# joeyee/Onet

Measured on AMD Instinct MI355X. Metric: training images/sec (twin 256x256 pass), higher is better.
Workload: dtype f32

## Files before the change

### onet_amd/csrc/conv_split.hip

```cpp
#include <algorithm>
#include <cstdlib>
#include "common.hpp"

using namespace onet;

typedef float f32x16 __attribute__((ext_vector_type(16)));
typedef __bf16 bf16x8 __attribute__((ext_vector_type(8)));
typedef __bf16 bf16x2 __attribute__((ext_vector_type(2)));
typedef unsigned int u32x4s __attribute__((ext_vector_type(4)));
typedef float f32x4s __attribute__((ext_vector_type(4)));

namespace {

constexpr unsigned OOB_S = 0x80000000u;

__device__ __forceinline__ __amdgpu_buffer_rsrc_t s_rsrc(const void* base, int64_t bytes) {
    const int n = bytes > 0x7fffffffll ? 0x7fffffff : (int)bytes;
    return __builtin_amdgcn_make_buffer_rsrc(const_cast<void*>(base), 0, n, 0x00020000);
}
__device__ __forceinline__ void split2(float a, float b, unsigned& hi, unsigned& mid) {
    const bf16x2 h = {(__bf16)a, (__bf16)b};
    const bf16x2 m = {(__bf16)(a - (float)h[0]), (__bf16)(b - (float)h[1])};
    hi = __builtin_bit_cast(unsigned, h);
    mid = __builtin_bit_cast(unsigned, m);
// ... 358 lines not shown
                (void)tap;
#pragma unroll
                for (int m = 0; m < 2; ++m)
#pragma unroll
                    for (int n = 0; n < NT; ++n) {
                        if constexpr (F16) {
                            const f16x8 ah = __builtin_bit_cast(f16x8, Aq[idx & 1][m][0]), am = __builtin_bit_cast(f16x8, Aq[idx & 1][m][1]);
                            const f16x8 bh = __builtin_bit_cast(f16x8, Bq[kx & 1][n + ky][0]), bm = __builtin_bit_cast(f16x8, Bq[kx & 1][n + ky][1]);
                            acc[m][n] = __builtin_amdgcn_mfma_f32_32x32x16_f16(am, bh, acc[m][n], 0, 0, 0);
                            acc[m][n] = __builtin_amdgcn_mfma_f32_32x32x16_f16(ah, bm, acc[m][n], 0, 0, 0);
                            acc[m][n] = __builtin_amdgcn_mfma_f32_32x32x16_f16(ah, bh, acc[m][n], 0, 0, 0);
                        } else {
                            const bf16x8 ah = __builtin_bit_cast(bf16x8, Aq[idx & 1][m][0]), am = __builtin_bit_cast(bf16x8, Aq[idx & 1][m][1]);
                            const bf16x8 bh = __builtin_bit_cast(bf16x8, Bq[kx & 1][n + ky][0]), bm = __builtin_bit_cast(bf16x8, Bq[kx & 1][n + ky][1]);
                            acc[m][n] = __builtin_amdgcn_mfma_f32_32x32x16_bf16(am, bh, acc[m][n], 0, 0, 0);
                            acc[m][n] = __builtin_amdgcn_mfma_f32_32x32x16_bf16(ah, bm, acc[m][n], 0, 0, 0);
                            acc[m][n] = __builtin_amdgcn_mfma_f32_32x32x16_bf16(ah, bh, acc[m][n], 0, 0, 0);
                        }
                    }
                __builtin_amdgcn_sched_barrier(0);
            }
            __syncthreads();
            buf ^= 1;
        }

        if constexpr (F16) {
#pragma unroll
            for (int m = 0; m < 2; ++m)
#pragma unroll
                for (int n = 0; n < NT; ++n)
#pragma unroll
                    for (int r = 0; r < 16; ++r) acc[m][n][r] *= acc_scale;
        }
        const auto [co0, tx, ty, b, y0, x0] = sp_tile(tile, a.coTiles, a.tilesX, a.tilesY);
        if constexpr (ST) {
            float* sc = reinterpret_cast<float*>(lds + 2 * BUF);
            constexpr float npw = (float)(NT * 32), inv_npw = 1.f / npw;
#pragma unroll
            for (int m = 0; m < 2; ++m)
#pragma unroll
                for (int r = 0; r < 16; ++r) {
                    const int piv = __builtin_bit_cast(int, acc[m][0][r]);
                    const float p0 = __builtin_bit_cast(float, __builtin_amdgcn_readlane(piv, 0));
                    const float p1 = __builtin_bit_cast(float, __builtin_amdgcn_readlane(piv, 32));
                    const float pv = kh ? p1 : p0;
                    float s1 = 0.f, s2 = 0.f;
#pragma unroll
                    for (int n = 0; n < NT; ++n) {
                        const float d = acc[m][n][r] - pv;
                        s1 += d;
                        s2 = fmaf(d, d, s2);
                    }
                    s1 = sp_half_sum(s1);
                    s2 = sp_half_sum(s2);
                    if (l31 == 31) {
                        const int cl = m * 32 + (r & 3) + 8 * (r >> 2) + 4 * kh;
                        sc[(wn * 64 + cl) * 2] = fmaf(s1, inv_npw, pv);
                        sc[(wn * 64 + cl) * 2 + 1] = fmaxf(fmaf(-s1 * inv_npw, s1, s2), 0.f);
                    }
                }
            __syncthreads();
            if (tid < 64 && co0 + tid < a.Cout) {
                float mw[8], qw[8];
#pragma unroll
                for (int w = 0; w < 8; ++w) {
                    mw[w] = sc[(w * 64 + tid) * 2];
                    qw[w] = sc[(w * 64 + tid) * 2 + 1];
                }
                const float mean = 0.125f * (((mw[0] + mw[1]) + (mw[2] + mw[3])) + ((mw[4] + mw[5]) + (mw[6] + mw[7])));
                float m2 = ((qw[0] + qw[1]) + (qw[2] + qw[3])) + ((qw[4] + qw[5]) + (qw[6] + qw[7]));
#pragma unroll
                for (int w = 0; w < 8; ++w) m2 = fmaf(npw * (mw[w] - mean), mw[w] - mean, m2);
                const int64_t nblk = (int64_t)a.B * a.tilesY * a.tilesX;
                const int64_t blk = ((int64_t)b * a.tilesY + ty) * a.tilesX + tx;
                float* sp = a.stats + ((int64_t)(co0 + tid) * nblk + blk) * 3;
                sp[0] = 8.f * npw;
                sp[1] = mean;
                sp[2] = m2;
            }
            __syncthreads();
        }
        float* zb = a.z + (int64_t)b * a.z_bs;
        const int xo = x0 + l31;
#pragma unroll
        for (int m = 0; m < 2; ++m)
#pragma unroll
            for (int n = 0; n < NT; ++n) {
                const int yo = y0 + wn * NT + n;
                if (yo < a.H && xo < a.W) {
#pragma unroll
                    for (int r = 0; r < 16; ++r) {
                        const int co = co0 + m * 32 + (r & 3) + 8 * (r >> 2) + 4 * kh;
                        if (co < a.Cout) zb[(int64_t)co * HW + (int64_t)yo * a.W + xo] = acc[m][n][r];
                    }
                }
            }
    }
}


typedef int i32x4s __attribute__((ext_vector_type(4)));
__device__ __forceinline__ i32x4s sp_rsrc4(const void* base, int64_t bytes) {
    const uint64_t p = reinterpret_cast<uint64_t>(base);
    i32x4s r;
    r.x = (int)(p & 0xffffffffu);
    r.y = (int)((p >> 32) & 0xffffu);
    r.z = bytes > 0x7fffffffll ? 0x7fffffff : (int)bytes;
    r.w = 0x00020000;
    return r;
}
__device__ __forceinline__ void sp_dma16(i32x4s rsrc, unsigned lds_base, unsigned voff, unsigned soff) {
    unsigned keep;
    asm volatile("s_nop 4\n\ts_mov_b32 %0, m0\n\ts_mov_b32 m0, %3\n\ts_nop 0\n\tbuffer_load_dwordx4 %1, %2, %4 offen lds\n\ts_mov_b32 m0, %0"
                 : "=&s"(keep)
                 : "v"(voff), "s"(rsrc), "s"(lds_base), "s"(soff)
                 : "memory");
}

__global__ void split_pack_act_kernel(const float* __restrict__ x, int64_t x_bs, unsigned* __restrict__ xs, int64_t xs_bs, int B, int C8,
                                      int H, int W, int f16, float scale, const unsigned* __restrict__ slots) {
    if (slots) {
        float inv;
        scale *= amax_scale(amax_read(slots), false, inv);
    }
    const int64_t n = (int64_t)B * C8 * H * W;
    for (int64_t i = blockIdx.x * (int64_t)blockDim.x + threadIdx.x; i < n; i += (int64_t)gridDim.x * blockDim.x) {
        const int xx = (int)(i % W);
        int64_t r = i / W;
        const int y = (int)(r % H);
        r /= H;
        const int c8 = (int)(r % C8), b = (int)(r / C8);
        const float* src = x + (int64_t)b * x_bs + ((int64_t)c8 * 8 * H + y) * W + xx;
        u32x4s hi, mid;
#pragma unroll
        for (int c = 0; c < 4; ++c) {
            const float va = src[(int64_t)(2 * c) * H * W] * scale, vb = src[(int64_t)(2 * c + 1) * H * W] * scale;
            unsigned h, m;
            if (f16 == 1) split2h(va, vb, h, m);
            else split2(va, vb, h, m);
            hi[c] = h;
            mid[c] = m;
        }
        if (f16 == 2) {
            reinterpret_cast<u32x4s*>(xs + (int64_t)b * xs_bs)[((int64_t)c8 * H + y) * W + xx] = hi;
            continue;
        }
        u32x4s* dst = reinterpret_cast<u32x4s*>(xs + (int64_t)b * xs_bs) + (((int64_t)c8 * H + y) * 2) * W + xx;
        dst[0] = hi;
        dst[W] = mid;
    }
}

struct SpPreArgs {
    const void* xs;
    int64_t xs_bs;
    const __bf16* wq;
    float* z;
    int64_t z_bs;
    int B, Cin, Cout, H, W, tilesX, tilesY, coTiles;
    float* stats;
    const unsigned* x_slots;
    int x_always;
    const unsigned* x_slots2;
    int split_ch;
    const float* rd_z = nullptr;
    int64_t rd_z_bs = 0;
    const float* rd_save = nullptr;
    int rd_gimg = 0;
    float* rd_rec = nullptr;
    unsigned* rd_amax = nullptr;
    int z16 = 0, rd_z16 = 0;
    void* zP = nullptr;
    int64_t zP_bs = 0;
    int zP_ch0 = 0;
    const unsigned* zP_slots = nullptr;
    const float* act_save = nullptr;
    unsigned* act_amax = nullptr;
    float* act_a = nullptr;
    int64_t act_a_bs = 0;
    const float* hd_L = nullptr;
    int64_t hd_L_bs = 0;
    float* hd_V = nullptr;
};

template <bool W16> struct SpPreCfg {
    static constexpr int NW = 8, NT = 16 / NW, TW = 32, CO_T = 64, ROWS = NW * NT;
    static constexpr int IN_ROWS = ROWS + 2, IN_COLS = W16 ? 36 : 34;
    static constexpr int NPIX = IN_ROWS * IN_COLS;
    static constexpr int NPIXP = W16 ? 656 : 640;
    static constexpr int W_PART = 9 * 2 * CO_T, W_SLOTS = 2 * W_PART, NWI = (W_SLOTS + NW * 64 - 1) / (NW * 64);
    static constexpr int IN_PART = 2 * NPIXP;
    static constexpr int BUF_SLOTS = W_SLOTS + 2 * IN_PART;
    static constexpr int LDS_BYTES = 2 * BUF_SLOTS * 16;
    static constexpr int NB = (NT - 1) + 3;
    static constexpr int LAST_TAP = 4;
    static_assert(CO_T == SpCfg::CO_T && ROWS == SpCfg::ROWS && TW == SpCfg::TW, "sp_tile: one tile shape for every kernel of the family");
};
template <bool ST, int PM, bool W16, bool ACT = false>
__global__ __launch_bounds__(SpPreCfg<W16>::NW * 64, SpPreCfg<W16>::NW / 4) void conv3x3_split_pre_kernel(SpPreArgs a) {
    constexpr bool F16 = PM == 1;
    static_assert(!ACT || (PM == 1 && !ST && !W16), "conv3x3_split_pre_kernel: the activation epilogue goes with the fp16 slot store");
    using C = SpPreCfg<W16>;
    constexpr int NT = C::NT, IN_COLS = C::IN_COLS, NWI = C::NWI, CO_T = C::CO_T, NPIXP = C::NPIXP, NB = C::NB;
    constexpr int BUF = C::BUF_SLOTS, W_PART = C::W_PART, IN_PART = C::IN_PART;
    constexpr int NWV = C::NW, NTH = NWV * 64;
    constexpr int NII = (2 * IN_PART + NTH - 1) / NTH;
    extern __shared__ __attribute__((aligned(16))) unsigned char smem_s[];
    u32x4s* lds = reinterpret_cast<u32x4s*>(smem_s);

    int t_first, t_end, t_stride;
    sp_tile_range(a.tilesX * a.tilesY * a.B * a.coTiles, t_first, t_end, t_stride);
    if (t_first >= t_end) return;

    const int tid = threadIdx.x, lane = tid & 63, wn = __builtin_amdgcn_readfirstlane(tid >> 6);
    const int l31 = lane & 31, kh = lane >> 5;
    const int HW = a.H * a.W;
    const int nchunks = PM == 2 ? a.Cin >> 5 : a.Cin >> 4;

    const i32x4s wr = sp_rsrc4(a.wq, (int64_t)a.Cin * (PM == 2 ? 1 : 2) * 9 * a.Cout * 2);
    float xs_inv = 1.f, xs_inv2 = 1.f;
    (void)amax_scale(amax_read(a.x_slots), a.x_always != 0, xs_inv);
    (void)amax_scale(amax_read(a.x_slots2), a.x_always != 0, xs_inv2);
    const int split_chunk = a.split_ch ? (PM == 2 ? a.split_ch >> 5 : a.split_ch >> 4) : 0;
    const float grp_ratio = split_chunk ? xs_inv / xs_inv2 : 1.f;
    const float acc_scale = (split_chunk ? xs_inv2 : xs_inv) * (F16 ? reinterpret_cast<const float*>(a.wq + (int64_t)a.Cin * 2 * 9 * a.Cout)[1] : 1.f);
    const unsigned in_step = (unsigned)(16 * HW * 4), w_step = (unsigned)(2 * 9 * 2 * a.Cout * 16);
    const unsigned lds0 = (unsigned)(uintptr_t)(__attribute__((address_space(3))) unsigned char*)smem_s;

    unsigned in_off[NII], w_off[NWI];
    i32x4s xr;
    int st_tile = t_first, st_chunk = 0;
    unsigned cin_bytes = 0, cw_bytes = 0;
    auto setup_stage = [&]() __attribute__((always_inline)) {
        const bool live = st_tile < t_end;
        const auto [co0, tx, ty, b, y0, x0] = sp_tile(live ? st_tile : t_first, a.coTiles, a.tilesX, a.tilesY);
        xr = sp_rsrc4(reinterpret_cast<const unsigned*>(a.xs) + (int64_t)(W16 ? 2 * b : b) * a.xs_bs,
                      (W16 ? a.xs_bs * 4 : 0) + (int64_t)a.Cin * HW * (PM == 2 ? 2 : 4));
#pragma unroll
        for (int k = 0; k < NII; ++k) {
            const int i = (wn + NWV * k) * 64 + lane;
            const int ph = i / NPIXP, pix = i % NPIXP;
            const int r = pix / IN_COLS, c = pix % IN_COLS;
            const int img = W16 ? c / 18 : 0;
            const int yy = y0 - 1 + r, xx = W16 ? c % 18 - 1 : x0 - 1 + c;
            const bool ok = live && i < 2 * IN_PART && pix < C::NPIX && yy >= 0 && yy < a.H && xx >= 0 && xx < a.W;
            const unsigned io = W16 ? (unsigned)(img * a.xs_bs * 4) : 0u;
            in_off[k] = !ok ? OOB_S : PM == 2 ? io + (unsigned)(((ph * a.H + yy) * a.W + xx) * 16)
                                              : io + (unsigned)(((((ph & 1) * a.H + yy) * 2 + (ph >> 1)) * a.W + xx) * 16);
        }
#pragma unroll
        for (int k = 0; k < NWI; ++k) {
            const int i = tid + NTH * k;
            const int co = i & (CO_T - 1), pth = i >> 6;
            const bool ok = live && (i < C::W_SLOTS) && (co0 + co < a.Cout);
            w_off[k] = ok ? (unsigned)((pth * a.Cout + co0 + co) * 16) : OOB_S;
        }
    };
    auto advance = [&]() __attribute__((always_inline)) {
        ++st_chunk;
        cin_bytes += in_step;
        cw_bytes += w_step;
        if (st_chunk == nchunks) {
            st_chunk = 0;
            cin_bytes = cw_bytes = 0;
            st_tile += t_stride;
            setup_stage();
        }
    };
    auto dma_in = [&](int buf, int k) __attribute__((always_inline)) {
        if ((wn + NWV * k) * 64 < 2 * IN_PART)
            sp_dma16(xr, lds0 + (unsigned)((buf * BUF + C::W_SLOTS + (wn + NWV * k) * 64) * 16), in_off[k], cin_bytes);
    };
    auto dma_w = [&](int buf, int k) __attribute__((always_inline)) {
        if (k < NWI - 1 || wn < (C::W_SLOTS - NTH * (NWI - 1)) / 64)
            sp_dma16(wr, lds0 + (unsigned)((buf * BUF + (wn + NWV * k) * 64) * 16), w_off[k], cw_bytes);
    };

    const u32x4s* const a_ptr = lds + kh * CO_T + l31;
    const u32x4s* const b_ptr = lds + C::W_SLOTS + kh * NPIXP + (wn * NT) * IN_COLS + (W16 ? (l31 >> 4) * 18 + (l31 & 15) : l31);

    setup_stage();
#pragma unroll
    for (int k = 0; k < NII; ++k) dma_in(0, k);
#pragma unroll
    for (int k = 0; k < NWI; ++k) dma_w(0, k);
    asm volatile("s_waitcnt vmcnt(0)" ::: "memory");
    __syncthreads();
    int buf = 0;
    float zP_scale = 1.f;
    if constexpr (PM == 1 && !ST && !W16) {
        float zinv;
        if (a.zP) zP_scale = amax_scale(amax_read(a.zP_slots), !ACT, zinv);
    }
    [[maybe_unused]] float* const act_cf = reinterpret_cast<float*>(lds + 2 * BUF);
    [[maybe_unused]] float cf_next = 0.f;
    [[maybe_unused]] int cf_par = 0;
    auto act_fetch = [&](int t) __attribute__((always_inline)) {
        if (tid < 192 && t < t_end) {
            const int k = tid >> 6;
            cf_next = a.act_save[(int64_t)(k + (k > 0)) * a.Cout + sp_tile(t, a.coTiles, a.tilesX, a.tilesY).co0 + (tid & 63)];
        }
    };
    if constexpr (ACT) act_fetch(t_first);
    for (int tile = t_first; tile < t_end; tile += t_stride) {
        if constexpr (ACT) {
            cf_par ^= 1;
            if (tid < 192) act_cf[cf_par * 192 + tid] = cf_next;
            act_fetch(tile + t_stride);
        }
        f32x16 acc[2][NT];
#pragma unroll
        for (int m = 0; m < 2; ++m)
#pragma unroll
            for (int n = 0; n < NT; ++n)
#pragma unroll
                for (int r = 0; r < 16; ++r) acc[m][n][r] = 0.f;

        for (int c = 0; c < nchunks; ++c) {
            if (split_chunk && c == split_chunk && grp_ratio != 1.f) {
#pragma unroll
                for (int m = 0; m < 2; ++m)
#pragma unroll
                    for (int n = 0; n < NT; ++n)
#pragma unroll
                        for (int r = 0; r < 16; ++r) acc[m][n][r] *= grp_ratio;
            }
            const u32x4s* const ab = a_ptr + buf * BUF;
            const u32x4s* const bb = b_ptr + buf * BUF;
            u32x4s Aq[2][2][2], Bq[2][NB][2];
#pragma unroll
            for (int j = 0; j < NB; ++j) {
                Bq[0][j][0] = bb[j * IN_COLS];
                Bq[0][j][1] = bb[j * IN_COLS + IN_PART];
            }
#pragma unroll
            for (int m = 0; m < 2; ++m) {
                Aq[0][m][0] = ab[m * 32];
                Aq[0][m][1] = ab[m * 32 + W_PART];
            }
#pragma unroll
            for (int idx = 0; idx < 9; ++idx) {
                const int kx = idx / 3, ky = idx % 3;
                if (idx < 8) {
                    const int nt = ((idx + 1) % 3) * 3 + (idx + 1) / 3;
#pragma unroll
                    for (int m = 0; m < 2; ++m) {
                        Aq[(idx + 1) & 1][m][0] = ab[nt * 2 * CO_T + m * 32];
                        Aq[(idx + 1) & 1][m][1] = ab[nt * 2 * CO_T + m * 32 + W_PART];
                    }
                }
                if (kx < 2) {
#pragma unroll
                    for (int j = 0; j < NB; ++j)
                        if (j % 3 == ky) {
                            Bq[(kx + 1) & 1][j][0] = bb[j * IN_COLS + kx + 1];
                            Bq[(kx + 1) & 1][j][1] = bb[j * IN_COLS + kx + 1 + IN_PART];
                        }
                }
                if (idx == 0) advance();
                {
                    constexpr int NPIECE = NII + NWI, PER = (NPIECE + C::LAST_TAP) / (C::LAST_TAP + 1);
#pragma unroll
                    for (int q = 0; q < PER; ++q) {
                        const int pc = idx * PER + q;
                        if (idx <= C::LAST_TAP && pc < NPIECE) {
                            if (pc & 1) { if (pc / 2 < NWI) dma_w(buf ^ 1, pc / 2); else dma_in(buf ^ 1, pc - NWI); }
                            else { if (pc / 2 < NII) dma_in(buf ^ 1, pc / 2); else dma_w(buf ^ 1, pc - NII); }
                        }
                    }
                }
                __builtin_amdgcn_sched_barrier(0);
#pragma unroll
                for (int m = 0; m < 2; ++m)
#pragma unroll
                    for (int n = 0; n < NT; ++n) {
                        if constexpr (PM == 2) {
                            const bf16x8 a0 = __builtin_bit_cast(bf16x8, Aq[idx & 1][m][0]), a1 = __builtin_bit_cast(bf16x8, Aq[idx & 1][m][1]);
                            const bf16x8 b0 = __builtin_bit_cast(bf16x8, Bq[kx & 1][n + ky][0]), b1 = __builtin_bit_cast(bf16x8, Bq[kx & 1][n + ky][1]);
                            acc[m][n] = __builtin_amdgcn_mfma_f32_32x32x16_bf16(a0, b0, acc[m][n], 0, 0, 0);
                            acc[m][n] = __builtin_amdgcn_mfma_f32_32x32x16_bf16(a1, b1, acc[m][n], 0, 0, 0);
                        } else if constexpr (F16) {
                            const f16x8 ah = __builtin_bit_cast(f16x8, Aq[idx & 1][m][0]), am = __builtin_bit_cast(f16x8, Aq[idx & 1][m][1]);
                            const f16x8 bh = __builtin_bit_cast(f16x8, Bq[kx & 1][n + ky][0]), bm = __builtin_bit_cast(f16x8, Bq[kx & 1][n + ky][1]);
                            acc[m][n] = __builtin_amdgcn_mfma_f32_32x32x16_f16(am, bh, acc[m][n], 0, 0, 0);
                            acc[m][n] = __builtin_amdgcn_mfma_f32_32x32x16_f16(ah, bm, acc[m][n], 0, 0, 0);
                            acc[m][n] = __builtin_amdgcn_mfma_f32_32x32x16_f16(ah, bh, acc[m][n], 0, 0, 0);
                        } else {
                            const bf16x8 ah = __builtin_bit_cast(bf16x8, Aq[idx & 1][m][0]), am = __builtin_bit_cast(bf16x8, Aq[idx & 1][m][1]);
                            const bf16x8 bh = __builtin_bit_cast(bf16x8, Bq[kx & 1][n + ky][0]), bm = __builtin_bit_cast(bf16x8, Bq[kx & 1][n + ky][1]);
                            acc[m][n] = __builtin_amdgcn_mfma_f32_32x32x16_bf16(am, bh, acc[m][n], 0, 0, 0);
                            acc[m][n] = __builtin_amdgcn_mfma_f32_32x32x16_bf16(ah, bm, acc[m][n], 0, 0, 0);
                            acc[m][n] = __builtin_amdgcn_mfma_f32_32x32x16_bf16(ah, bh, acc[m][n], 0, 0, 0);
                        }
                    }
                __builtin_amdgcn_sched_barrier(0);
            }
            asm volatile("s_waitcnt vmcnt(0)" ::: "memory");
            __syncthreads();
            buf ^= 1;
        }

#pragma unroll
        for (int m = 0; m < 2; ++m)
#pragma unroll
            for (int n = 0; n < NT; ++n)
#pragma unroll
                for (int r = 0; r < 16; ++r) acc[m][n][r] *= acc_scale;
        const auto [co0, tx, ty, b, y0, x0] = sp_tile(tile, a.coTiles, a.tilesX, a.tilesY);
        if constexpr (ST) {
            float* sc = reinterpret_cast<float*>(lds + 2 * BUF);
            constexpr float npw = (float)(NT * 32), inv_npw = 1.f / npw;
#pragma unroll
            for (int m = 0; m < 2; ++m)
#pragma unroll
                for (int r = 0; r < 16; ++r) {
                    const int piv = __builtin_bit_cast(int, acc[m][0][r]);
                    const float p0 = __builtin_bit_cast(float, __builtin_amdgcn_readlane(piv, 0));
                    const float p1 = __builtin_bit_cast(float, __builtin_amdgcn_readlane(piv, 32));
                    const float pv = kh ? p1 : p0;
                    float s1 = 0.f, s2 = 0.f;
#pragma unroll
                    for (int n = 0; n < NT; ++n) {
                        const float d = acc[m][n][r] - pv;
                        s1 += d;
                        s2 = fmaf(d, d, s2);
                    }
                    s1 = sp_half_sum(s1);
                    s2 = sp_half_sum(s2);
                    if (l31 == 31) {
                        const int cl = m * 32 + (r & 3) + 8 * (r >> 2) + 4 * kh;
                        sc[(wn * 64 + cl) * 2] = fmaf(s1, inv_npw, pv);
                        sc[(wn * 64 + cl) * 2 + 1] = fmaxf(fmaf(-s1 * inv_npw, s1, s2), 0.f);
                    }
                }
            __syncthreads();
            if (tid < 64 && co0 + tid < a.Cout) {
                float mw[8], qw[8];
#pragma unroll
                for (int w = 0; w < 8; ++w) {
                    mw[w] = sc[(w * 64 + tid) * 2];
                    qw[w] = sc[(w * 64 + tid) * 2 + 1];
                }
                const float mean = 0.125f * (((mw[0] + mw[1]) + (mw[2] + mw[3])) + ((mw[4] + mw[5]) + (mw[6] + mw[7])));
                float m2 = ((qw[0] + qw[1]) + (qw[2] + qw[3])) + ((qw[4] + qw[5]) + (qw[6] + qw[7]));
#pragma unroll
                for (int w = 0; w < 8; ++w) m2 = fmaf(npw * (mw[w] - mean), mw[w] - mean, m2);
                const int64_t nblk = (int64_t)a.B * a.tilesY * a.tilesX;
                const int64_t blk = ((int64_t)b * a.tilesY + ty) * a.tilesX + tx;
                float* sp = a.stats + ((int64_t)(co0 + tid) * nblk + blk) * 3;
                sp[0] = 8.f * npw;
                sp[1] = mean;
                sp[2] = m2;
            }
            __syncthreads();
        }
        float* zb = a.z + (int64_t)(W16 ? 2 * b + (l31 >> 4) : b) * a.z_bs;
        const int xo = W16 ? (l31 & 15) : x0 + l31;
        if constexpr (ACT) {
            const float* cf = act_cf + cf_par * 192;
            float vmax = 0.f;
#pragma unroll
            for (int m = 0; m < 2; ++m)
#pragma unroll
                for (int g = 0; g < 4; ++g) {
                    const int cl = m * 32 + 8 * g + 4 * kh;
                    const f32x4s mean = *reinterpret_cast<const f32x4s*>(cf + cl);
                    const f32x4s sc = *reinterpret_cast<const f32x4s*>(cf + 64 + cl);
                    const f32x4s sh = *reinterpret_cast<const f32x4s*>(cf + 128 + cl);
#pragma unroll
                    for (int n = 0; n < NT; ++n)
#pragma unroll
                        for (int j = 0; j < 4; ++j) {
                            const float v = fmaxf(fmaf(acc[m][n][4 * g + j] - mean[j], sc[j], sh[j]), 0.f);
                            acc[m][n][4 * g + j] = v;
                            vmax = fmaxf(vmax, v);
                        }
                }
            if (a.act_amax) {
#pragma unroll
                for (int o = 32; o > 0; o >>= 1) vmax = fmaxf(vmax, __shfl_xor(vmax, o, 64));
                if (lane == 0 && vmax == vmax)
                    atomicMax(a.act_amax + ((tile * NWV + wn) & (AMAX_SLOTS - 1)) * AMAX_STRIDE, __builtin_bit_cast(unsigned, vmax));
            }
            if (a.act_a) {
                float* ab = a.act_a + (int64_t)b * a.act_a_bs;
#pragma unroll
                for (int m = 0; m < 2; ++m)
#pragma unroll
                    for (int n = 0; n < NT; ++n) {
                        const int yo = y0 + wn * NT + n;
                        if (yo < a.H && xo < a.W) {
#pragma unroll
                            for (int r = 0; r < 16; ++r) {
                                const int co = co0 + m * 32 + (r & 3) + 8 * (r >> 2) + 4 * kh;
                                if (co < a.Cout) ab[(int64_t)co * HW + (int64_t)yo * a.W + xo] = acc[m][n][r];
                            }
                        }
                    }
            }
        }
        if constexpr (PM == 1 && !ST && !W16) {
            if (ACT || (a.zP && co0 >= a.zP_ch0)) {
                const float zs = zP_scale;
                u32x4s* zp = reinterpret_cast<u32x4s*>(reinterpret_cast<unsigned*>(a.zP) + (int64_t)b * a.zP_bs);
#pragma unroll
                for (int m = 0; m < 2; ++m)
#pragma unroll
                    for (int n = 0; n < NT; ++n) {
                        const int yo = y0 + wn * NT + n;
#pragma unroll
                        for (int e = 0; e < 2; ++e) {
                            float v[8];
#pragma unroll
                            for (int j = 0; j < 4; ++j) {
                                const float f0 = acc[m][n][8 * e + j], f1 = acc[m][n][8 * e + 4 + j];
                                const unsigned d0 = __builtin_bit_cast(unsigned, f0);
                                const unsigned d1 = __builtin_bit_cast(unsigned, f1);
                                const auto sw = __builtin_amdgcn_permlane32_swap(d0, d1, false, false);
                                const unsigned lo = sw[0], hi4 = sw[1];
                                v[j] = __builtin_bit_cast(float, lo);
                                v[4 + j] = __builtin_bit_cast(float, hi4);
                            }
                            u32x4s hi, mid;
#pragma unroll
                            for (int k = 0; k < 4; ++k) {
                                unsigned hh, mm;
                                split2h_s(v[2 * k], v[2 * k + 1], zs, hh, mm);
                                hi[k] = hh;
                                mid[k] = mm;
                            }
                            if (yo < a.H && xo < a.W) {
                                const int c8 = ((co0 - a.zP_ch0 + m * 32) >> 3) + 2 * e + kh;
                                u32x4s* d = zp + ((int64_t)(c8 * a.H + yo) * 2) * a.W + xo;
                                d[0] = hi;
                                d[a.W] = mid;
                            }
                        }
                    }
                continue;
            }
        }
#pragma unroll
        for (int m = 0; m < 2; ++m)
#pragma unroll
            for (int n = 0; n < NT; ++n) {
                const int yo = y0 + wn * NT + n;
                if (yo < a.H && xo < a.W) {
#pragma unroll
                    for (int r = 0; r < 16; ++r) {
                        const int co = co0 + m * 32 + (r & 3) + 8 * (r >> 2) + 4 * kh;
                        if (co < a.Cout) zb[(int64_t)co * HW + (int64_t)yo * a.W + xo] = acc[m][n][r];
                    }
                }
            }
    }
}


template <int CTRL> __device__ __forceinline__ float dpp_add(float x) {
    return x + __builtin_bit_cast(float, __builtin_amdgcn_update_dpp(0, __builtin_bit_cast(int, x), CTRL, 0xf, 0xf, false));
}
template <bool ST, int PM, bool W16, bool RD = false, bool ACT = false, bool HEAD = false>
__global__ __launch_bounds__(512, 2) void conv3x3_pre16_kernel(SpPreArgs a) {
    constexpr bool F16 = PM == 1;
    static_assert(!ACT || (PM == 2 && !ST && !W16 && !RD), "conv3x3_pre16_kernel: the activation epilogue goes with the one-part bf16 slot store");
    static_assert(!HEAD || (PM != 0 && !ST && !W16 && !RD && !ACT), "conv3x3_pre16_kernel: the head epilogue replaces every store of a plain forward launch");
    using C = SpPreCfg<W16>;
    static_assert(C::NW == 8 && C::NT == 2, "conv3x3_pre16_kernel: 8 waves of 2 rows");
    constexpr int NT = 2, IN_COLS = C::IN_COLS, NWI = C::NWI, CO_T = C::CO_T, NPIXP = C::NPIXP;
    constexpr int BUF = C::BUF_SLOTS, IN_PART = C::IN_PART;
    constexpr int NII = (2 * IN_PART + 511) / 512;
    constexpr int CH_OFF = W16 ? 18 : 16;
    constexpr int NSTEP = PM == 2 ? 9 : 14;
    extern __shared__ __attribute__((aligned(16))) unsigned char smem_s[];
    u32x4s* lds = reinterpret_cast<u32x4s*>(smem_s);

    int t_first, t_end, t_stride;
    sp_tile_range(a.tilesX * a.tilesY * a.B * a.coTiles, t_first, t_end, t_stride);
    if (t_first >= t_end) return;

    const int tid = threadIdx.x, lane = tid & 63, wn = __builtin_amdgcn_readfirstlane(tid >> 6);
    const int r16 = lane & 15, lq = lane >> 4, hq = lq & 1, gq = lq >> 1;
    const int HW = a.H * a.W;
    const int nchunks = PM == 2 ? a.Cin >> 5 : a.Cin >> 4;

    const i32x4s wr = sp_rsrc4(a.wq, (int64_t)a.Cin * (PM == 2 ? 1 : 2) * 9 * a.Cout * 2);
    float xs_inv = 1.f, xs_inv2 = 1.f;
    (void)amax_scale(amax_read(a.x_slots), a.x_always != 0, xs_inv);
    (void)amax_scale(amax_read(a.x_slots2), a.x_always != 0, xs_inv2);
    const int split_chunk = a.split_ch ? (PM == 2 ? a.split_ch >> 5 : a.split_ch >> 4) : 0;
    const float grp_ratio = split_chunk ? xs_inv / xs_inv2 : 1.f;
    const float acc_scale = (split_chunk ? xs_inv2 : xs_inv) * (F16 ? reinterpret_cast<const float*>(a.wq + (int64_t)a.Cin * 2 * 9 * a.Cout)[1] : 1.f);
    const unsigned in_step = (unsigned)(16 * HW * 4), w_step = (unsigned)(2 * 9 * 2 * a.Cout * 16);
    const unsigned lds0 = (unsigned)(uintptr_t)(__attribute__((address_space(3))) unsigned char*)smem_s;

    unsigned in_off[NII], w_off[NWI];
    i32x4s xr;
    int st_tile = t_first, st_chunk = 0;
    unsigned cin_bytes = 0, cw_bytes = 0;
    auto setup_stage = [&]() __attribute__((always_inline)) {
        const bool live = st_tile < t_end;
        const auto [co0, tx, ty, b, y0, x0] = sp_tile(live ? st_tile : t_first, a.coTiles, a.tilesX, a.tilesY);
        xr = sp_rsrc4(reinterpret_cast<const unsigned*>(a.xs) + (int64_t)(W16 ? 2 * b : b) * a.xs_bs,
                      (W16 ? a.xs_bs * 4 : 0) + (int64_t)a.Cin * HW * (PM == 2 ? 2 : 4));
#pragma unroll
        for (int k = 0; k < NII; ++k) {
            const int i = (wn + 8 * k) * 64 + lane;
            const int ph = i / NPIXP, pix = i % NPIXP;
            const int r = pix / IN_COLS, c = pix % IN_COLS;
            const int img = W16 ? c / 18 : 0;
            const int yy = y0 - 1 + r, xx = W16 ? c % 18 - 1 : x0 - 1 + c;
            const bool ok = live && i < 2 * IN_PART && pix < C::NPIX && yy >= 0 && yy < a.H && xx >= 0 && xx < a.W;
            const unsigned io = W16 ? (unsigned)(img * a.xs_bs * 4) : 0u;
            in_off[k] = !ok ? OOB_S : PM == 2 ? io + (unsigned)(((ph * a.H + yy) * a.W + xx) * 16)
                                              : io + (unsigned)(((((ph & 1) * a.H + yy) * 2 + (ph >> 1)) * a.W + xx) * 16);
        }
#pragma unroll
        for (int k = 0; k < NWI; ++k) {
            const int i = tid + 512 * k;
            const int co = i & (CO_T - 1), pth = i >> 6;
            const bool ok = live && (i < C::W_SLOTS) && (co0 + co < a.Cout);
            w_off[k] = ok ? (unsigned)((pth * a.Cout + co0 + co) * 16) : OOB_S;
        }
    };
    auto advance = [&]() __attribute__((always_inline)) {
        ++st_chunk;
        cin_bytes += in_step;
        cw_bytes += w_step;
        if (st_chunk == nchunks) {
            st_chunk = 0;
            cin_bytes = cw_bytes = 0;
            st_tile += t_stride;
            setup_stage();
        }
    };
    auto dma_in = [&](int buf, int k) __attribute__((always_inline)) {
        if ((wn + 8 * k) * 64 < 2 * IN_PART)
            sp_dma16(xr, lds0 + (unsigned)((buf * BUF + C::W_SLOTS + (wn + 8 * k) * 64) * 16), in_off[k], cin_bytes);
    };
    auto dma_w = [&](int buf, int k) __attribute__((always_inline)) {
        if (k < NWI - 1 || wn < (C::W_SLOTS - 512 * (NWI - 1)) / 64)
            sp_dma16(wr, lds0 + (unsigned)((buf * BUF + (wn + 8 * k) * 64) * 16), w_off[k], cw_bytes);
    };

    const int xrow0 = (wn * NT) * IN_COLS + r16;
    const u32x4s* const xa_p = lds + C::W_SLOTS + (PM == 2 ? lq : hq) * NPIXP + xrow0;
    const u32x4s* const xh_p = lds + C::W_SLOTS + (2 + hq) * NPIXP + xrow0 + gq;
    const u32x4s* const xv_p = lds + C::W_SLOTS + (2 + hq) * NPIXP + xrow0 + gq * IN_COLS + 2;
    const u32x4s* const xs_p = lds + C::W_SLOTS + (2 + hq) * NPIXP + xrow0 + 2;
    const u32x4s* const wa_p = lds + (gq * 9 * 2 + hq) * CO_T + r16;
    const u32x4s* const wh_p = lds + (gq * 2 + hq) * CO_T + r16;
    const u32x4s* const wv_p = lds + ((3 * gq + 2) * 2 + hq) * CO_T + r16;
    const u32x4s* const ws_p = gq == 0 ? lds + (8 * 2 + hq) * CO_T + r16 : lds + C::W_SLOTS + C::NPIX;
    const int ws_ct = gq == 0 ? 16 : 0;

    setup_stage();
#pragma unroll
    for (int k = 0; k < NII; ++k) dma_in(0, k);
#pragma unroll
    for (int k = 0; k < NWI; ++k) dma_w(0, k);
    asm volatile("s_waitcnt vmcnt(0)" ::: "memory");
    __syncthreads();
    int buf = 0;
    [[maybe_unused]] float* const act_cf = reinterpret_cast<float*>(lds + 2 * BUF);
    [[maybe_unused]] float cf_next = 0.f;
    [[maybe_unused]] int cf_par = 0;
    auto act_fetch = [&](int t) __attribute__((always_inline)) {
        if (tid < 192 && t < t_end) {
            const int k = tid >> 6;
            cf_next = a.act_save[(int64_t)(k + (k > 0)) * a.Cout + sp_tile(t, a.coTiles, a.tilesX, a.tilesY).co0 + (tid & 63)];
        }
    };
    if constexpr (ACT || HEAD) act_fetch(t_first);
    for (int tile = t_first; tile < t_end; tile += t_stride) {
        if constexpr (ACT || HEAD) {
            cf_par ^= 1;
            if (tid < 192) act_cf[cf_par * 192 + tid] = cf_next;
            act_fetch(tile + t_stride);
        }
        f32x4s acc[4][NT][2];
#pragma unroll
        for (int ct = 0; ct < 4; ++ct)
#pragma unroll
            for (int n = 0; n < NT; ++n)
#pragma unroll
                for (int ch = 0; ch < 2; ++ch) acc[ct][n][ch] = f32x4s{0.f, 0.f, 0.f, 0.f};

        for (int c = 0; c < nchunks; ++c) {
            if (split_chunk && c == split_chunk && grp_ratio != 1.f) {
#pragma unroll
                for (int ct = 0; ct < 4; ++ct)
#pragma unroll
                    for (int n = 0; n < NT; ++n)
#pragma unroll
                        for (int ch = 0; ch < 2; ++ch) acc[ct][n][ch] *= grp_ratio;
            }
            const int bo = buf * BUF;
            u32x4s Xp[2][NT + 2][2], Wf[2][4];
            auto load_x = [&](int ph, int f) __attribute__((always_inline)) {
                const int j = f >> 1, ch = f & 1, p = ph & 1;
                if (ph < 3) Xp[p][j][ch] = xa_p[bo + j * IN_COLS + ch * CH_OFF + ph];
                else if (ph == 3) Xp[p][j][ch] = xh_p[bo + j * IN_COLS + ch * CH_OFF];
                else if (j < NT) Xp[p][j][ch] = xv_p[bo + j * IN_COLS + ch * CH_OFF];
                else Xp[p][j][ch] = xs_p[bo + j * IN_COLS + ch * CH_OFF];
            };
            auto load_w = [&](int s) __attribute__((always_inline)) {
#pragma unroll
                for (int ct = 0; ct < 4; ++ct) {
                    if (s < 9) Wf[s & 1][ct] = wa_p[bo + ((s % 3) * 3 + s / 3) * 2 * CO_T + ct * 16];
                    else if (s < 12) Wf[s & 1][ct] = wh_p[bo + (s - 9) * 6 * CO_T + ct * 16];
                    else if (s == 12) Wf[s & 1][ct] = wv_p[bo + ct * 16];
                    else Wf[s & 1][ct] = ws_p[bo + ct * ws_ct];
                }
            };
#pragma unroll
            for (int f = 0; f < 2 * (NT + 2); ++f) load_x(0, f);
            load_w(0);
#pragma unroll
            for (int s = 0; s < NSTEP; ++s) {
                const int ph = s < 9 ? s / 3 : (s < 12 ? 3 : 4);
                const int ro = s < 9 ? s % 3 : (s < 12 ? s - 9 : (s == 12 ? 0 : NT));
                if (s + 1 < NSTEP) load_w(s + 1);
                if (s < 12 && ph + 1 < (PM == 2 ? 3 : 5)) {
#pragma unroll
                    for (int f = 0; f < 2 * (NT + 2); ++f)
                        if (f % 3 == s % 3) load_x(ph + 1, f);
                }
                if (s == 0) advance();
                {
                    constexpr int NPIECE = NII + NWI, PER = (NPIECE + C::LAST_TAP) / (C::LAST_TAP + 1);
#pragma unroll
                    for (int q = 0; q < PER; ++q) {
                        const int pc = s * PER + q;
                        if (s <= C::LAST_TAP && pc < NPIECE) {
                            if (pc & 1) { if (pc / 2 < NWI) dma_w(buf ^ 1, pc / 2); else dma_in(buf ^ 1, pc - NWI); }
                            else { if (pc / 2 < NII) dma_in(buf ^ 1, pc / 2); else dma_w(buf ^ 1, pc - NII); }
                        }
                    }
                }
                __builtin_amdgcn_sched_barrier(0);
#pragma unroll
                for (int ct = 0; ct < 4; ++ct)
#pragma unroll
                    for (int n = 0; n < NT; ++n)
#pragma unroll
                        for (int ch = 0; ch < 2; ++ch) {
                            if constexpr (F16)
                                acc[ct][n][ch] = __builtin_amdgcn_mfma_f32_16x16x32_f16(__builtin_bit_cast(f16x8, Xp[ph & 1][ro + n][ch]),
                                                                                        __builtin_bit_cast(f16x8, Wf[s & 1][ct]), acc[ct][n][ch], 0, 0, 0);
                            else
                                acc[ct][n][ch] = __builtin_amdgcn_mfma_f32_16x16x32_bf16(__builtin_bit_cast(bf16x8, Xp[ph & 1][ro + n][ch]),
                                                                                         __builtin_bit_cast(bf16x8, Wf[s & 1][ct]), acc[ct][n][ch], 0, 0, 0);
                        }
                __builtin_amdgcn_sched_barrier(0);
            }
            asm volatile("s_waitcnt vmcnt(0)" ::: "memory");
            __syncthreads();
            buf ^= 1;
        }

#pragma unroll
        for (int ct = 0; ct < 4; ++ct)
#pragma unroll
            for (int n = 0; n < NT; ++n)
#pragma unroll
                for (int ch = 0; ch < 2; ++ch) acc[ct][n][ch] *= acc_scale;
        const auto [co0, tx, ty, b, y0, x0] = sp_tile(tile, a.coTiles, a.tilesX, a.tilesY);
        if constexpr (ST) {
            float* sc = reinterpret_cast<float*>(lds + (buf ^ 1) * BUF);
            constexpr float npw = (float)(NT * 32);
#pragma unroll
            for (int ct = 0; ct < 4; ++ct) {
                const float pv = acc[ct][0][0][0];
                float s1 = 0.f, s2 = 0.f;
#pragma unroll
                for (int n = 0; n < NT; ++n)
#pragma unroll
                    for (int ch = 0; ch < 2; ++ch)
#pragma unroll
                        for (int r = 0; r < 4; ++r) {
                            const float d = acc[ct][n][ch][r] - pv;
                            s1 += d;
                            s2 = fmaf(d, d, s2);
                        }
                float mean = fmaf(s1, 1.f / 16.f, pv), m2 = fmaxf(fmaf(-s1 * (1.f / 16.f), s1, s2), 0.f), cnt = 16.f;
#pragma unroll
                for (int o = 16; o <= 32; o <<= 1) {
                    const float mo = __shfl_xor(mean, o, 64), qo = __shfl_xor(m2, o, 64);
                    const float dlt = mo - mean;
                    m2 = (m2 + qo) + (0.5f * cnt) * dlt * dlt;
                    mean = 0.5f * (mean + mo);
                    cnt *= 2.f;
                }
                if (lq == 0) {
                    sc[(wn * 64 + ct * 16 + r16) * 2] = mean;
                    sc[(wn * 64 + ct * 16 + r16) * 2 + 1] = m2;
                }
            }
            __syncthreads();
            if (tid < 64 && co0 + tid < a.Cout) {
                float mw[8], qw[8];
#pragma unroll
                for (int w = 0; w < 8; ++w) {
                    mw[w] = sc[(w * 64 + tid) * 2];
                    qw[w] = sc[(w * 64 + tid) * 2 + 1];
                }
                const float mean = 0.125f * (((mw[0] + mw[1]) + (mw[2] + mw[3])) + ((mw[4] + mw[5]) + (mw[6] + mw[7])));
                float m2 = ((qw[0] + qw[1]) + (qw[2] + qw[3])) + ((qw[4] + qw[5]) + (qw[6] + qw[7]));
#pragma unroll
                for (int w = 0; w < 8; ++w) m2 = fmaf(npw * (mw[w] - mean), mw[w] - mean, m2);
                const int64_t nblk = (int64_t)a.B * a.tilesY * a.tilesX;
                const int64_t blk = ((int64_t)b * a.tilesY + ty) * a.tilesX + tx;
                float* sp = a.stats + ((int64_t)(co0 + tid) * nblk + blk) * 3;
                sp[0] = 8.f * npw;
                sp[1] = mean;
                sp[2] = m2;
            }
            __syncthreads();
        }
        if constexpr (ACT) {
            const float* cf = act_cf + cf_par * 192;
            float vmax = 0.f;
#pragma unroll
            for (int ct = 0; ct < 4; ++ct) {
                const float mean = cf[ct * 16 + r16], sc = cf[64 + ct * 16 + r16], sh = cf[128 + ct * 16 + r16];
#pragma unroll
                for (int n = 0; n < NT; ++n)
#pragma unroll
                    for (int ch = 0; ch < 2; ++ch)
#pragma unroll
                        for (int r = 0; r < 4; ++r) {
                            const float v = fmaxf(fmaf(acc[ct][n][ch][r] - mean, sc, sh), 0.f);
                            acc[ct][n][ch][r] = v;
                            vmax = fmaxf(vmax, v);
                        }
            }
            if (a.act_amax) {
#pragma unroll
                for (int o = 32; o > 0; o >>= 1) vmax = fmaxf(vmax, __shfl_xor(vmax, o, 64));
                if (lane == 0 && vmax == vmax)
                    atomicMax(a.act_amax + ((tile * 8 + wn) & (AMAX_SLOTS - 1)) * AMAX_STRIDE, __builtin_bit_cast(unsigned, vmax));
            }
        }
        if constexpr (HEAD) {
            f32x4s lr[4][NT][2];
            const float* Lb = a.hd_L + (int64_t)b * a.hd_L_bs;
#pragma unroll
            for (int ct = 0; ct < 4; ++ct)
#pragma unroll
                for (int n = 0; n < NT; ++n)
#pragma unroll
                    for (int ch = 0; ch < 2; ++ch) {
                        const int co = co0 + ct * 16 + r16, yo = y0 + wn * NT + n, xo = x0 + 16 * ch + 4 * lq;
                        f32x4s ll = {0.f, 0.f, 0.f, 0.f};
                        if (co < a.Cout && yo < a.H && xo < a.W) ll = *reinterpret_cast<const f32x4s*>(Lb + (int64_t)co * HW + (int64_t)yo * a.W + xo);
                        lr[ct][n][ch] = ll;
                    }
            __builtin_amdgcn_sched_barrier(0);
            const float* cf = act_cf + cf_par * 192;
            f32x4s v[NT][2];
#pragma unroll
            for (int n = 0; n < NT; ++n)
#pragma unroll
                for (int ch = 0; ch < 2; ++ch) v[n][ch] = f32x4s{0.f, 0.f, 0.f, 0.f};
#pragma unroll
            for (int ct = 0; ct < 4; ++ct) {
                const float mean = cf[ct * 16 + r16], sc = cf[64 + ct * 16 + r16], sh = cf[128 + ct * 16 + r16];
#pragma unroll
                for (int n = 0; n < NT; ++n)
#pragma unroll
                    for (int ch = 0; ch < 2; ++ch)
#pragma unroll
                        for (int r = 0; r < 4; ++r)
                            v[n][ch][r] = fmaf(lr[ct][n][ch][r], fmaxf(fmaf(acc[ct][n][ch][r] - mean, sc, sh), 0.f), v[n][ch][r]);
            }
#pragma unroll
            for (int n = 0; n < NT; ++n)
#pragma unroll
                for (int ch = 0; ch < 2; ++ch)
#pragma unroll
                    for (int r = 0; r < 4; ++r)
                        v[n][ch][r] = dpp_add<0x140>(dpp_add<0x141>(dpp_add<0x4E>(dpp_add<0xB1>(v[n][ch][r]))));
            float* Vb = a.hd_V + (int64_t)b * HW;
#pragma unroll
            for (int n = 0; n < NT; ++n)
#pragma unroll
                for (int ch = 0; ch < 2; ++ch) {
                    const int yo = y0 + wn * NT + n, xo = x0 + 16 * ch + 4 * lq;
                    if (r16 == 2 * n + ch && yo < a.H && xo < a.W) *reinterpret_cast<f32x4s*>(Vb + (int64_t)yo * a.W + xo) = v[n][ch];
                }
            continue;
        }
        f32x4s zr[4][NT][2];
        const float* rd_sv = nullptr;
        if constexpr (RD) {
            const int img0 = W16 ? 2 * b : b;
            rd_sv = a.rd_save + (int64_t)(a.rd_gimg ? img0 / a.rd_gimg : 0) * 4 * a.Cout;
#pragma unroll
            for (int ct = 0; ct < 4; ++ct)
#pragma unroll
                for (int n = 0; n < NT; ++n)
#pragma unroll
                    for (int ch = 0; ch < 2; ++ch) {
                        const int co = co0 + ct * 16 + r16, yo = y0 + wn * NT + n, xo = (W16 ? 0 : x0 + 16 * ch) + 4 * lq;
                        f32x4s zz = {0.f, 0.f, 0.f, 0.f};
                        if (co < a.Cout && yo < a.H && xo < a.W) {
                            const int64_t zo = (int64_t)(W16 ? img0 + ch : img0) * a.rd_z_bs + (int64_t)co * HW + (int64_t)yo * a.W + xo;
                            if (a.rd_z16) {
                                const uint2 u = *reinterpret_cast<const uint2*>(reinterpret_cast<const __bf16*>(a.rd_z) + zo);
                                zz = f32x4s{__builtin_bit_cast(float, u.x << 16), __builtin_bit_cast(float, u.x & 0xffff0000u),
                                            __builtin_bit_cast(float, u.y << 16), __builtin_bit_cast(float, u.y & 0xffff0000u)};
                            } else {
                                zz = *reinterpret_cast<const f32x4s*>(a.rd_z + zo);
                            }
                        }
                        zr[ct][n][ch] = zz;
                    }
            __builtin_amdgcn_sched_barrier(0);
        }
        {
            const int half = r16 >> 3, c8 = r16 & 7;
            float* zb = a.z + (int64_t)(W16 ? 2 * b + half : b) * a.z_bs;
            const int xo = (W16 ? 0 : x0 + 16 * half) + 4 * lq;
#pragma unroll
            for (int n = 0; n < NT; ++n) {
                const int yo = y0 + wn * NT + n;
#pragma unroll
                for (int ct = 0; ct < 4; ++ct) {
                    const i32x4s va = __builtin_bit_cast(i32x4s, acc[ct][n][0]), vb = __builtin_bit_cast(i32x4s, acc[ct][n][1]);
                    const i32x4s e1 = {__builtin_amdgcn_update_dpp(va.x, vb.x, 0x128, 0xf, 0xc, false), __builtin_amdgcn_update_dpp(va.y, vb.y, 0x128, 0xf, 0xc, false),
                                       __builtin_amdgcn_update_dpp(va.z, vb.z, 0x128, 0xf, 0xc, false), __builtin_amdgcn_update_dpp(va.w, vb.w, 0x128, 0xf, 0xc, false)};
                    const i32x4s e2 = {__builtin_amdgcn_update_dpp(vb.x, va.x, 0x128, 0xf, 0x3, false), __builtin_amdgcn_update_dpp(vb.y, va.y, 0x128, 0xf, 0x3, false),
                                       __builtin_amdgcn_update_dpp(vb.z, va.z, 0x128, 0xf, 0x3, false), __builtin_amdgcn_update_dpp(vb.w, va.w, 0x128, 0xf, 0x3, false)};
                    const f32x4s d1 = __builtin_bit_cast(f32x4s, e1), d2 = __builtin_bit_cast(f32x4s, e2);
                    if constexpr (PM == 2 && !ST && !W16 && !RD) {
                        if constexpr (ACT) {
                            if (a.act_a && yo < a.H && xo < a.W) {
                                const int co = co0 + ct * 16 + c8;
                                float* o = a.act_a + (int64_t)b * a.act_a_bs + (int64_t)co * HW + (int64_t)yo * a.W + xo;
                                if (co < a.Cout) *reinterpret_cast<f32x4s*>(o) = d1;
                                if (co + 8 < a.Cout) *reinterpret_cast<f32x4s*>(o + (int64_t)8 * HW) = d2;
                            }
                        }
                        if (ACT || (a.zP && co0 >= a.zP_ch0)) {
                            const unsigned a0 = pack2bf(d1[0], d1[1]), a1 = pack2bf(d1[2], d1[3]);
                            const unsigned b0 = pack2bf(d2[0], d2[1]), b1 = pack2bf(d2[2], d2[3]);
                            const bool o1 = (c8 & 1) != 0, o2 = (c8 & 2) != 0, o4 = (c8 & 4) != 0;
                            auto st1 = [&](unsigned x) {
                                const unsigned y = (unsigned)__shfl_xor((int)x, 1, 64);
                                return o1 ? ((y >> 16) | (x & 0xffff0000u)) : ((x & 0xffffu) | (y << 16));
                            };
                            const unsigned A0 = st1(a0), A1 = st1(a1), B0 = st1(b0), B1 = st1(b1);
                            const unsigned ra = (unsigned)__shfl_xor((int)(o2 ? A0 : A1), 2, 64), rb = (unsigned)__shfl_xor((int)(o2 ? B0 : B1), 2, 64);
                            const unsigned ka = o2 ? A1 : A0, kb = o2 ? B1 : B0;
                            const unsigned Alo = o2 ? ra : ka, Ahi = o2 ? ka : ra, Blo = o2 ? rb : kb, Bhi = o2 ? kb : rb;
                            const unsigned r0 = (unsigned)__shfl_xor((int)(o4 ? Alo : Blo), 4, 64), r1 = (unsigned)__shfl_xor((int)(o4 ? Ahi : Bhi), 4, 64);
                            const u32x4s slot = o4 ? u32x4s{r0, r1, Blo, Bhi} : u32x4s{Alo, Ahi, r0, r1};
                            const int xs = x0 + 16 * half + 4 * lq + (c8 & 3);
                            if (yo < a.H && xs < a.W) {
                                const int g8 = ((co0 - a.zP_ch0) >> 3) + 2 * ct + (o4 ? 1 : 0);
                                u32x4s* zp = reinterpret_cast<u32x4s*>(reinterpret_cast<unsigned*>(a.zP) + (int64_t)b * a.zP_bs);
                                zp[((int64_t)g8 * a.H + yo) * a.W + xs] = slot;
                            }
                            continue;
                        }
                    }
                    if (yo < a.H && xo < a.W) {
                        const int co = co0 + ct * 16 + c8;
                        const int64_t off = (int64_t)co * HW + (int64_t)yo * a.W + xo;
                        if (a.z16) {
                            __bf16* o = reinterpret_cast<__bf16*>(a.z) + (int64_t)(W16 ? 2 * b + half : b) * a.z_bs + off;
                            const bf16x2 p0 = {(__bf16)d1[0], (__bf16)d1[1]}, p1 = {(__bf16)d1[2], (__bf16)d1[3]};
                            const bf16x2 q0 = {(__bf16)d2[0], (__bf16)d2[1]}, q1 = {(__bf16)d2[2], (__bf16)d2[3]};
                            if (co < a.Cout) *reinterpret_cast<uint2*>(o) = uint2{__builtin_bit_cast(unsigned, p0), __builtin_bit_cast(unsigned, p1)};
                            if (co + 8 < a.Cout) *reinterpret_cast<uint2*>(o + (int64_t)8 * HW) = uint2{__builtin_bit_cast(unsigned, q0), __builtin_bit_cast(unsigned, q1)};
                        } else {
                            float* o = zb + off;
                            if (co < a.Cout) *reinterpret_cast<f32x4s*>(o) = d1;
                            if (co + 8 < a.Cout) *reinterpret_cast<f32x4s*>(o + (int64_t)8 * HW) = d2;
                        }
                    }
                }
            }
        }
        if constexpr (RD) {
            __builtin_amdgcn_sched_barrier(0);
            float* sc = reinterpret_cast<float*>(lds + (buf ^ 1) * BUF);
            float vmax = 0.f;
#pragma unroll
            for (int ct = 0; ct < 4; ++ct) {
                const int co = co0 + ct * 16 + r16, cc = min(co, a.Cout - 1);
                const float mean = rd_sv[cc], invstd = rd_sv[a.Cout + cc], scl = rd_sv[2 * a.Cout + cc], sh = rd_sv[3 * a.Cout + cc];
                float s1 = 0.f, s2 = 0.f;
#pragma unroll
                for (int n = 0; n < NT; ++n)
#pragma unroll
                    for (int ch = 0; ch < 2; ++ch) {
                        const int yo = y0 + wn * NT + n, xo = (W16 ? 0 : x0 + 16 * ch) + 4 * lq;
                        if (co < a.Cout && yo < a.H && xo < a.W) {
#pragma unroll
                            for (int r = 0; r < 4; ++r) {
                                const float da = acc[ct][n][ch][r], d = zr[ct][n][ch][r] - mean;
                                const float dy = fmaf(d, scl, sh) > 0.f ? da : 0.f;
                                s1 += dy;
                                s2 = fmaf(dy, d * invstd, s2);
                                vmax = fmaxf(vmax, fabsf(da));
                            }
                        }
                    }
                s1 += __shfl_xor(s1, 16, 64);
                s2 += __shfl_xor(s2, 16, 64);
                s1 += __shfl_xor(s1, 32, 64);
                s2 += __shfl_xor(s2, 32, 64);
                if (lq == 0) {
                    sc[(wn * 64 + ct * 16 + r16) * 2] = s1;
                    sc[(wn * 64 + ct * 16 + r16) * 2 + 1] = s2;
                }
            }
            if (a.rd_amax) {
#pragma unroll
                for (int o = 32; o > 0; o >>= 1) vmax = fmaxf(vmax, __shfl_xor(vmax, o, 64));
                if (lane == 0 && vmax == vmax) atomicMax(a.rd_amax + ((blockIdx.x * 8 + wn) & (AMAX_SLOTS - 1)) * AMAX_STRIDE, __builtin_bit_cast(unsigned, vmax));
            }
            __syncthreads();
            if (tid < 64 && co0 + tid < a.Cout) {
                double t1 = 0.0, t2 = 0.0;
#pragma unroll
                for (int w = 0; w < 8; ++w) {
                    t1 += (double)sc[(w * 64 + tid) * 2];
                    t2 += (double)sc[(w * 64 + tid) * 2 + 1];
                }
                const int64_t blk = ((int64_t)b * a.tilesY + ty) * a.tilesX + tx;
                float* o = a.rd_rec + (blk * a.Cout + co0 + tid) * 4;
                o[0] = (float)t1;
                o[1] = (float)(t1 - (double)o[0]);
                o[2] = (float)t2;
                o[3] = (float)(t2 - (double)o[2]);
            }
            __syncthreads();
        }
    }
}

template <class Args>
int sp_launch_persistent(void (*kern)(Args), PerDeviceOnce& once, int lds_bytes, int64_t tiles, int block, const char* name, const Args& a, hipStream_t st) {
    if (once.first()) {
        (void)hipFuncSetAttribute(reinterpret_cast<const void*>(kern), hipFuncAttributeMaxDynamicSharedMemorySize, lds_bytes);
    }
    const int64_t resident = (int64_t)device_cu_count();
    const int64_t blocks = std::min<int64_t>((tiles + 7) / 8 * 8, std::max<int64_t>(8, resident / 8 * 8));
    hipLaunchKernelGGL(kern, dim3((unsigned)blocks), dim3(block), lds_bytes, st, a);
    return check_launch(name);
}

template <bool ST, int PM, bool W16, bool RD = false, bool ACT = false, bool HEAD = false>
int launch_split_pre(SpPreArgs a, hipStream_t st) {
    using C = SpPreCfg<W16>;
    const int LDS_BYTES = C::LDS_BYTES + (ST ? C::NW * 64 * 2 * 4 : 0) + (ACT || HEAD ? 2 * 3 * 64 * 4 : 0);
    a.tilesX = W16 ? 1 : cdiv(a.W, C::TW);
    a.tilesY = cdiv(a.H, C::ROWS);
// ... 990 lines not shown
```

Measured before the change: 575.4.

## Prefetch next chunk's first LDS fragments before last tap's MFMAs

Moves the end-of-chunk wait and barrier into the last tap iteration of both conv split kernels. Right after that barrier, the first A/B (or X/W) register fragments for the next chunk are loaded from the other LDS buffer, and the MFMAs of the last tap then run over those loads. This hides the LDS read latency that otherwise sat at the start of each chunk. In exchange it adds register pressure, because the fragment arrays now live across chunks, and it relies on the last tap issuing no DMA, which is checked with static_asserts.

```diff
diff --git a/onet_amd/csrc/conv_split.hip b/onet_amd/csrc/conv_split.hip
--- a/onet_amd/csrc/conv_split.hip
+++ b/onet_amd/csrc/conv_split.hip
@@ -684,6 +684,20 @@
         }
     };
     if constexpr (ACT) act_fetch(t_first);
+    u32x4s Aq[2][2][2], Bq[2][NB][2];
+    auto load_first = [&](int bo) __attribute__((always_inline)) {
+#pragma unroll
+        for (int j = 0; j < NT; ++j) {
+            Bq[0][j][0] = b_ptr[bo + j * IN_COLS];
+            Bq[0][j][1] = b_ptr[bo + j * IN_COLS + IN_PART];
+        }
+#pragma unroll
+        for (int m = 0; m < 2; ++m) {
+            Aq[1][m][0] = a_ptr[bo + m * 32];
+            Aq[1][m][1] = a_ptr[bo + m * 32 + W_PART];
+        }
+    };
+    load_first(0);
     for (int tile = t_first; tile < t_end; tile += t_stride) {
         if constexpr (ACT) {
             cf_par ^= 1;
@@ -707,18 +721,18 @@
 #pragma unroll
                         for (int r = 0; r < 16; ++r) acc[m][n][r] *= grp_ratio;
             }
+            static_assert(8 > C::LAST_TAP + 1, "the last tap issues no DMA, and every piece is taps old there");
             const u32x4s* const ab = a_ptr + buf * BUF;
             const u32x4s* const bb = b_ptr + buf * BUF;
-            u32x4s Aq[2][2][2], Bq[2][NB][2];
-#pragma unroll
-            for (int j = 0; j < NB; ++j) {
+#pragma unroll
+            for (int m = 0; m < 2; ++m) {
+                Aq[0][m][0] = Aq[1][m][0];
+                Aq[0][m][1] = Aq[1][m][1];
+            }
+#pragma unroll
+            for (int j = NT; j < NB; ++j) {
                 Bq[0][j][0] = bb[j * IN_COLS];
                 Bq[0][j][1] = bb[j * IN_COLS + IN_PART];
-            }
-#pragma unroll
-            for (int m = 0; m < 2; ++m) {
-                Aq[0][m][0] = ab[m * 32];
-                Aq[0][m][1] = ab[m * 32 + W_PART];
             }
 #pragma unroll
             for (int idx = 0; idx < 9; ++idx) {
@@ -750,6 +764,11 @@
                             else { if (pc / 2 < NII) dma_in(buf ^ 1, pc / 2); else dma_w(buf ^ 1, pc - NII); }
                         }
                     }
+                }
+                if (idx == 8) {
+                    asm volatile("s_waitcnt vmcnt(0) lgkmcnt(0)" ::: "memory");
+                    __syncthreads();
+                    load_first((buf ^ 1) * BUF);
                 }
                 __builtin_amdgcn_sched_barrier(0);
 #pragma unroll
@@ -777,8 +796,6 @@
                     }
                 __builtin_amdgcn_sched_barrier(0);
             }
-            asm volatile("s_waitcnt vmcnt(0)" ::: "memory");
-            __syncthreads();
             buf ^= 1;
         }
 
@@ -1054,6 +1071,29 @@
         }
     };
     if constexpr (ACT || HEAD) act_fetch(t_first);
+    u32x4s Xp[2][NT + 2][2], Wf[2][4];
+    auto load_x = [&](int bo, int ph, int f) __attribute__((always_inline)) {
+        const int j = f >> 1, ch = f & 1, p = ph & 1;
+        if (ph < 3) Xp[p][j][ch] = xa_p[bo + j * IN_COLS + ch * CH_OFF + ph];
+        else if (ph == 3) Xp[p][j][ch] = xh_p[bo + j * IN_COLS + ch * CH_OFF];
+        else if (j < NT) Xp[p][j][ch] = xv_p[bo + j * IN_COLS + ch * CH_OFF];
+        else Xp[p][j][ch] = xs_p[bo + j * IN_COLS + ch * CH_OFF];
+    };
+    auto load_w = [&](int bo, int s, int set) __attribute__((always_inline)) {
+#pragma unroll
+        for (int ct = 0; ct < 4; ++ct) {
+            if (s < 9) Wf[set][ct] = wa_p[bo + ((s % 3) * 3 + s / 3) * 2 * CO_T + ct * 16];
+            else if (s < 12) Wf[set][ct] = wh_p[bo + (s - 9) * 6 * CO_T + ct * 16];
+            else if (s == 12) Wf[set][ct] = wv_p[bo + ct * 16];
+            else Wf[set][ct] = ws_p[bo + ct * ws_ct];
+        }
+    };
+    auto load_first = [&](int bo) __attribute__((always_inline)) {
+#pragma unroll
+        for (int f = 0; f < 2 * NT; ++f) load_x(bo, 0, f);
+        load_w(bo, 0, NSTEP & 1);
+    };
+    load_first(0);
     for (int tile = t_first; tile < t_end; tile += t_stride) {
         if constexpr (ACT || HEAD) {
             cf_par ^= 1;
@@ -1077,36 +1117,23 @@
 #pragma unroll
                         for (int ch = 0; ch < 2; ++ch) acc[ct][n][ch] *= grp_ratio;
             }
+            static_assert(NSTEP - 1 > C::LAST_TAP + 1, "the last step issues no DMA, and every piece is steps old there");
             const int bo = buf * BUF;
-            u32x4s Xp[2][NT + 2][2], Wf[2][4];
-            auto load_x = [&](int ph, int f) __attribute__((always_inline)) {
-                const int j = f >> 1, ch = f & 1, p = ph & 1;
-                if (ph < 3) Xp[p][j][ch] = xa_p[bo + j * IN_COLS + ch * CH_OFF + ph];
-                else if (ph == 3) Xp[p][j][ch] = xh_p[bo + j * IN_COLS + ch * CH_OFF];
-                else if (j < NT) Xp[p][j][ch] = xv_p[bo + j * IN_COLS + ch * CH_OFF];
-                else Xp[p][j][ch] = xs_p[bo + j * IN_COLS + ch * CH_OFF];
-            };
-            auto load_w = [&](int s) __attribute__((always_inline)) {
-#pragma unroll
-                for (int ct = 0; ct < 4; ++ct) {
-                    if (s < 9) Wf[s & 1][ct] = wa_p[bo + ((s % 3) * 3 + s / 3) * 2 * CO_T + ct * 16];
-                    else if (s < 12) Wf[s & 1][ct] = wh_p[bo + (s - 9) * 6 * CO_T + ct * 16];
-                    else if (s == 12) Wf[s & 1][ct] = wv_p[bo + ct * 16];
-                    else Wf[s & 1][ct] = ws_p[bo + ct * ws_ct];
-                }
-            };
-#pragma unroll
-            for (int f = 0; f < 2 * (NT + 2); ++f) load_x(0, f);
-            load_w(0);
+            if constexpr (NSTEP & 1) {
+#pragma unroll
+                for (int ct = 0; ct < 4; ++ct) Wf[0][ct] = Wf[1][ct];
+            }
+#pragma unroll
+            for (int f = 2 * NT; f < 2 * (NT + 2); ++f) load_x(bo, 0, f);
 #pragma unroll
             for (int s = 0; s < NSTEP; ++s) {
                 const int ph = s < 9 ? s / 3 : (s < 12 ? 3 : 4);
                 const int ro = s < 9 ? s % 3 : (s < 12 ? s - 9 : (s == 12 ? 0 : NT));
-                if (s + 1 < NSTEP) load_w(s + 1);
+                if (s + 1 < NSTEP) load_w(bo, s + 1, (s + 1) & 1);
                 if (s < 12 && ph + 1 < (PM == 2 ? 3 : 5)) {
 #pragma unroll
                     for (int f = 0; f < 2 * (NT + 2); ++f)
-                        if (f % 3 == s % 3) load_x(ph + 1, f);
+                        if (f % 3 == s % 3) load_x(bo, ph + 1, f);
                 }
                 if (s == 0) advance();
                 {
@@ -1119,6 +1146,11 @@
                             else { if (pc / 2 < NII) dma_in(buf ^ 1, pc / 2); else dma_w(buf ^ 1, pc - NII); }
                         }
                     }
+                }
+                if (s == NSTEP - 1) {
+                    asm volatile("s_waitcnt vmcnt(0) lgkmcnt(0)" ::: "memory");
+                    __syncthreads();
+                    load_first((buf ^ 1) * BUF);
                 }
                 __builtin_amdgcn_sched_barrier(0);
 #pragma unroll
@@ -1136,8 +1168,6 @@
                         }
                 __builtin_amdgcn_sched_barrier(0);
             }
-            asm volatile("s_waitcnt vmcnt(0)" ::: "memory");
-            __syncthreads();
             buf ^= 1;
         }
 
```

New measurement: 579.2, median of 6. About the same (+0.7%).
